# jinlong17/DA-Detect

Measured on AMD Instinct MI355X. Metric: train images/sec, DA-Faster-RCNN R-50 Cityscapes->Foggy, higher is better.
Workload: dtype f32

## Files before the change

### da_detect_amd/_C.py

```python
import contextlib
import os
import ctypes
import time

import torch

from . import _lib
from . import amax as _amax
from ._lib import ConvDesc

CL = torch.channels_last

NMS_TIE_RULE = 0

PROFILER = None
_KNAME_CACHE = {}


class KernelProfiler(object):

    def __init__(self, pool=0, only=None):
        self.only = only
        self._pool = []
        for _ in range(pool):
# ... 831 lines not shown
    R, C, h, w = x.shape
    y = torch.empty((R, C), dtype=torch.float32, device=x.device)
    _lib.call("dadet_avgpool_forward", _p(x), _p(y), R, h * w, C, _stream())
    return _amax.carry(y, x)


def avgpool_backward(gy, h, w):
    _dev(gy, "gy")
    gy = gy.contiguous()
    R, C = gy.shape
    gx = torch.empty((R, C, h, w), dtype=torch.float32, device=gy.device, memory_format=CL)
    _lib.call("dadet_avgpool_backward", _p(gy), _p(gx), R, h * w, C, _stream())
    return _amax.carry(gx, gy)


def nchw3_to_nhwc4(x):
    _dev(x, "x")
    x = x.contiguous()
    N, C, H, W = x.shape
    assert C == 3
    y = torch.empty((N, 4, H, W), dtype=torch.float32, device=x.device, memory_format=CL)
    _lib.call("dadet_nchw3_to_nhwc4", _p(x), _p(y), N, H, W, _stream())
    if _mode4():
        _amax.ptr(x)
        _amax.carry(y, x)
    return y


def two_image_ends(r_cst, n_src):
    return min(max(int(n_src), 0), int(r_cst)), int(r_cst)
# ... 303 lines not shown
        _lib.call("dadet_fpn_merge_levels", arr, len(chunk), _stream())
    return outs


def fast_rcnn_loss(class_logits, box_regression, src, labels_src, rows_pos, map_inds, targets_pos):
    _dev(class_logits, "class_logits"), _dev(box_regression, "box_regression")
    cls, reg = class_logits.contiguous(), box_regression.contiguous()
    losses = torch.empty(2, dtype=torch.float32, device=cls.device)
    g_cls, g_reg = torch.zeros_like(cls), torch.zeros_like(reg)
    _lib.call("dadet_fast_rcnn_loss", _p(cls), _p(reg), cls.shape[1], reg.shape[1], _p(src.contiguous()),
              _p(labels_src.contiguous()), int(src.numel()), _p(rows_pos.contiguous()), _p(map_inds.contiguous()),
              _p(targets_pos.contiguous()), int(rows_pos.numel()), _p(losses), _p(g_cls), _p(g_reg), _stream())
    return losses, g_cls, g_reg


def fast_rcnn_loss_rows(class_logits, box_regression, loss_labels, regression_targets):
    _dev(class_logits, "class_logits"), _dev(box_regression, "box_regression")
    cls, reg = class_logits.contiguous(), box_regression.contiguous()
    R = cls.shape[0]
    if loss_labels.numel() != R or regression_targets.numel() != 4 * R or reg.shape[0] != R:
        raise _lib.DadetError("fast_rcnn_loss_rows: %d logit rows, %d labels, %d target values" % (
            R, loss_labels.numel(), regression_targets.numel()))
    losses = torch.empty(2, dtype=torch.float32, device=cls.device)
    g_cls, g_reg = torch.zeros_like(cls), torch.zeros_like(reg)
    _lib.call("dadet_fast_rcnn_loss_rows", _p(cls), _p(reg), R, cls.shape[1], reg.shape[1],
              _p(loss_labels.contiguous().to(torch.int64)), _p(_dev(regression_targets, "targets").contiguous()),
              _p(losses), _p(g_cls), _p(g_reg), _stream())
    return losses, g_cls, g_reg


SAMPLE_ROIS_MAX = 4096
PROPOSALS_SAMPLE_MAX_GT = 1024


def sample_rois_buffers(rows, device):
    return dict(idx=torch.empty(rows, dtype=torch.int64, device=device),
                objectness=torch.empty(rows, dtype=torch.float32, device=device),
                boxes=torch.empty((rows, 4), dtype=torch.float32, device=device),
                labels=torch.empty(rows, dtype=torch.int64, device=device),
# ... 331 lines not shown
```

### da_detect_amd/_lib.py

```python
import ctypes
import os
from ctypes import POINTER, c_char_p, c_float, c_int, c_int64, c_size_t, c_uint64, c_void_p

_HERE = os.path.dirname(os.path.abspath(__file__))
LIB_PATH = os.environ.get("DADET_LIB") or os.path.join(_HERE, "libdadet_hip.so")
_lib = None
DEFAULT_GEMM_MODE = "4"


class ConvDesc(ctypes.Structure):

    _fields_ = [(n, c_int) for n in (
        "N", "H", "W", "Cin", "Cout", "KH", "KW", "stride", "pad", "Ho", "Wo", "OutH", "OutW",
        "out_spatial_stride", "relu_mode")]


class ConvPlanInfo(ctypes.Structure):

    _fields_ = [(n, c_int) for n in (
        "family", "variant", "tiles_m", "tiles_n", "ksplit", "splits", "rows_per_split", "sk_dp_tiles", "sk_tiles", "sk_units",
        "sk_iters", "sk_max_parts", "big_splits", "big_body", "launches", "grid", "needs_counters")] + [
        ("workspace_bytes", c_size_t), ("name", ctypes.c_char * 64)]


# ... 127 lines not shown
    "dadet_roi_pool_backward": [_P, _P, _P, _P, c_int, c_int, c_int, c_int, c_int, c_int, c_int, _P],
    "dadet_deform_psroi_pool_forward": [_P, _P, _P, _P, _P, c_int, c_int, c_int, c_int, c_int, c_int, c_float,
                                        c_int, c_int, c_int, c_int, c_int, c_float, c_int, _P],
    "dadet_deform_psroi_pool_backward": [_P, _P, _P, _P, _P, _P, _P, c_int, c_int, c_int, c_int, c_int, c_int,
                                         c_float, c_int, c_int, c_int, c_int, c_int, c_float, c_int, _P],
    "dadet_relu_bn_backward": [_P, _P, _P, _P, _P, c_int64, c_int, _P],
    "dadet_relu_bn_backward_m": [_P, _P, _P, _P, _P, c_int64, c_int, _P, _P, _P],
    "dadet_colsum_workspace_bytes": [c_int64, c_int, POINTER(c_size_t)],
    "dadet_colsum": [_P, _P, c_int64, c_int, _P, c_size_t, _P],
    "dadet_colsum_ld": [_P, c_int, _P, c_int64, c_int, c_int, _P, c_size_t, _P],
    "dadet_channel_affine": [_P, _P, _P, _P, c_int64, c_int, c_int, _P],
    "dadet_maxpool3x3s2_forward": [_P, _P, c_int, c_int, c_int, c_int, c_int, c_int, _P],
    "dadet_maxpool3x3s2_relu_backward": [_P, _P, _P, _P, c_int, c_int, c_int, c_int, c_int, c_int, _P, _P],
    "dadet_avgpool_forward": [_P, _P, c_int, c_int, c_int, _P],
    "dadet_avgpool_backward": [_P, _P, c_int, c_int, c_int, _P],
    "dadet_nchw3_to_nhwc4": [_P, _P, c_int, c_int, c_int, _P],
    "dadet_rpn_decode_clip": [_P, _P, _P, c_int, c_float, c_float, c_float, c_float, c_float, c_float, c_float, _P, _P],
    "dadet_da_img_head_loss_forward": [_P, _P, _P, _P, _P, _P, c_int, c_int, c_int, _P],
    "dadet_da_img_head_loss_backward": [_P, _P, _P, _P, _P, _P, _P, _P, _P, c_int, c_int, c_int, _P],
    "dadet_da_img_head_loss_backward_g": [_P, _P, _P, _P, _P, _P, _P, c_float, c_float, _P, _P, _P, _P, c_int, c_int, c_int,
                                          _P],
    "dadet_da_img_head_loss_backward_gm": [_P, _P, _P, _P, _P, _P, _P, c_float, c_float, _P, _P, _P, _P, c_int, c_int, c_int,
                                          _P, _P, _P],
    "dadet_da_ins_tail_forward": [_P, _P, _P, _P, _P, _P, _P, c_int, c_int, c_int, c_int, c_int, _P],
    "dadet_da_ins_tail_backward": [_P, _P, _P, _P, _P, _P, c_float, _P, _P, _P, _P, c_int, c_int, c_int, c_int, c_int, _P],
    "dadet_da_ins_tail_forward_n": [_P, _P, _P, _P, _P, _P, _P, c_int, c_int, POINTER(c_int), c_int, c_int, c_int, _P],
    "dadet_da_ins_tail_backward_n": [_P, _P, _P, _P, _P, _P, c_float, _P, _P, _P, _P, c_int, c_int, POINTER(c_int), c_int,
                                     c_int, c_int, _P],
    "dadet_da_ins_dropout_rows": [_P, _P, _P, c_int64, c_int, _P],
    "dadet_da_ins_merge": [_P, _P, _P, _P, _P, _P, c_int64, c_int, _P],
# ... 45 lines not shown
```

### da_detect_amd/csrc/elementwise.hip

```cpp
#include "box_match.h"
#include "conv_common.h"
#include <float.h>

namespace dadet {

static inline int stream_blocks(int64_t work_items, int threads) {
  int64_t b = ceil_div64(work_items, threads);
  if (b > kMaxStreamBlocks) b = kMaxStreamBlocks;
  if (b < 1) b = 1;
  return (int)b;
}

__global__ void relu_bn_backward_kernel(const float4* __restrict__ g, const float4* __restrict__ y,
                                        const float4* __restrict__ scale, float4* __restrict__ g_out,
                                        float4* __restrict__ g_scaled, int64_t total4, int C4,
                                        unsigned* __restrict__ amax_out, unsigned* __restrict__ amax_scaled) {
  float mo = 0.f, ms = 0.f;
  for (int64_t i = (int64_t)blockIdx.x * blockDim.x + threadIdx.x; i < total4;
       i += (int64_t)gridDim.x * blockDim.x) {
    const float4 gv = g[i];
    float4 r = gv;
    if (y) {
      const float4 yv = y[i];
      r.x = yv.x > 0.f ? gv.x : 0.f;
      r.y = yv.y > 0.f ? gv.y : 0.f;
      r.z = yv.z > 0.f ? gv.z : 0.f;
      r.w = yv.w > 0.f ? gv.w : 0.f;
    }
    if (g_out) g_out[i] = r;
    mo = fmaxf(fmaxf(mo, fmaxf(fabsf(r.x), fabsf(r.y))), fmaxf(fabsf(r.z), fabsf(r.w)));
    if (g_scaled) {
      float4 s = r;
      if (scale) {
        const float4 sc = scale[i % C4];
        s.x *= sc.x; s.y *= sc.y; s.z *= sc.z; s.w *= sc.w;
      }
      g_scaled[i] = s;
      ms = fmaxf(fmaxf(ms, fmaxf(fabsf(s.x), fabsf(s.y))), fmaxf(fabsf(s.z), fabsf(s.w)));
    }
  }
  if (amax_out) amax_publish(amax_out, mo);
  if (amax_scaled) amax_publish(amax_scaled, ms);
}

__global__ __launch_bounds__(256) void colsum_partial_kernel(const float* __restrict__ g,
                                                             float* __restrict__ partial, int64_t rows,
                                                             int C, int64_t rows_per_split, int cb, int ld) {
  __shared__ float red[256];
  const int lanes = 256 / cb;
// ... 422 lines not shown
  DADET_REQUIRE(rows >= 0 && C > 0 && C % 4 == 0, "relu_bn_backward: C=%d must be a multiple of 4", C);
  if (rows == 0) return DADET_OK;
  DADET_REQUIRE(g && (g_out || g_scaled), "relu_bn_backward: null pointer");
  DADET_REQUIRE(aligned16(g) && aligned16(y) && aligned16(scale) && aligned16(g_out) && aligned16(g_scaled),
                "relu_bn_backward: pointers must be 16-byte aligned");
  const int64_t total4 = rows * (C / 4);
  hipLaunchKernelGGL(relu_bn_backward_kernel, dim3(stream_blocks(total4, 256)), dim3(256), 0,
                     as_stream(stream), reinterpret_cast<const float4*>(g),
                     reinterpret_cast<const float4*>(y), reinterpret_cast<const float4*>(scale),
                     reinterpret_cast<float4*>(g_out), reinterpret_cast<float4*>(g_scaled), total4, C / 4,
                     reinterpret_cast<unsigned*>(g_out ? amax_out : nullptr),
                     reinterpret_cast<unsigned*>(g_scaled ? amax_scaled : nullptr));
  return check_launch("relu_bn_backward");
}

extern "C" int dadet_colsum_workspace_bytes(int64_t rows, int C, size_t* bytes_out) {
  DADET_REQUIRE(rows >= 0 && C > 0 && bytes_out, "colsum_workspace_bytes: bad args");
  *bytes_out = rows == 0 ? 0 : sizeof(float) * (size_t)colsum_splits(rows, C) * C;
  return DADET_OK;
}

extern "C" int dadet_colsum_ld(const float* g, int ld, float* out, int64_t rows, int C, int accumulate, void* workspace,
                               size_t workspace_bytes, void* stream) {
  DADET_REQUIRE(rows >= 0 && C > 0 && ld >= C && out, "colsum: bad args (rows=%lld C=%d ld=%d)", (long long)rows, C, ld);
  hipStream_t st = as_stream(stream);
  if (rows == 0) {
    if (!accumulate) (void)hipMemsetAsync(out, 0, sizeof(float) * C, st);
    return check_launch("colsum(empty)");
  }
  DADET_REQUIRE(g, "colsum: null input");
// ... 186 lines not shown
```

### da_detect_amd/layers/misc.py

```python

import torch
from torch import nn
from torch.autograd import Function
from torch.autograd.function import once_differentiable

from .. import _C
from .. import amax as _amax
from .conv import conv2d_affine_act

CL = torch.channels_last


class FrozenBatchNorm2d(nn.Module):

    def __init__(self, n):
        super(FrozenBatchNorm2d, self).__init__()
        self.register_buffer("weight", torch.ones(n))
        self.register_buffer("bias", torch.zeros(n))
        self.register_buffer("running_mean", torch.zeros(n))
        self.register_buffer("running_var", torch.ones(n))
        self._cache = None

    def folded(self):
        key = (self.weight._version, self.bias._version, self.running_mean._version,
# ... 278 lines not shown


class _AvgPoolHW(Function):

    @staticmethod
    def forward(ctx, x):
        ctx.hw = (x.shape[2], x.shape[3])
        return _C.avgpool_forward(x)

    @staticmethod
    @once_differentiable
    def backward(ctx, g):
        return _C.avgpool_backward(g, *ctx.hw)


_POOL_MEMO = True


def global_avg_pool(x):
    if x.shape[0] == 0:
        return x.new_empty((0, x.shape[1]))
    memo = x.__dict__.get("_dadet_pooled") if _POOL_MEMO else None
    if memo is not None and memo[0] == x._version and memo[1] == torch.is_grad_enabled():
        return memo[2]
    y = _AvgPoolHW.apply(x)
    x._dadet_pooled = (x._version, torch.is_grad_enabled(), y)
    return y
```

### da_detect_amd/modeling/backbone/resnet.py

```python
from collections import namedtuple

import torch
import torch.nn.functional as F
from torch import nn

from ... import _C
from ...layers import Conv2d, FrozenBatchNorm2d, conv2d_affine_act
from ...utils.registry import Registry
from ...utils import streams
from ...utils.streams import WgradLane

StageSpec = namedtuple("StageSpec", ["index", "block_count", "return_features"])


def _specs(*rows):
    return tuple(StageSpec(index=i, block_count=c, return_features=r) for (i, c, r) in rows)


ResNet50StagesTo5 = _specs((1, 3, False), (2, 4, False), (3, 6, False), (4, 3, True))
ResNet50StagesTo4 = _specs((1, 3, False), (2, 4, False), (3, 6, True))
ResNet101StagesTo5 = _specs((1, 3, False), (2, 4, False), (3, 23, False), (4, 3, True))
ResNet101StagesTo4 = _specs((1, 3, False), (2, 4, False), (3, 23, True))
ResNet50FPNStagesTo5 = _specs((1, 3, True), (2, 4, True), (3, 6, True), (4, 3, True))
ResNet101FPNStagesTo5 = _specs((1, 3, True), (2, 4, True), (3, 23, True), (4, 3, True))
# ... 30 lines not shown
        reqs, batch = self.reqs, self.batch
        key = self.key + tuple((tuple(r["x"].shape), r["stride"]) for r in reqs)

        def run():
            ok = self._known.get(key, True) and _C.conv_wgrad_group(reqs, batch)
            if not ok:
                self._known[key] = self._known[self.key] = False
                for r in reqs:
                    _C.conv_wgrad(r["x"], r["gy"], r["weight_shape"], r["stride"], r["pad"], out_scale=r["out_scale"],
                                  dw=r["dw"], accumulate=True, pending=batch)

        self.lane.run_group(run, *[t for r in reqs for t in (r["x"], r["gy"])])
        self.reqs = []


class _BlockBackward(object):

    def __init__(self, needs, x, w1, wd, s1, sd, stride):
        self.need_x, self.n1, self.n2, self.n3, nd = needs
        self.nd = nd and wd is not None
        self.x, self.w1, self.wd, self.s1, self.sd, self.stride = x, w1, wd, s1, sd, stride

    def open(self, G, out, out_private, y2, w2, w3, s3):
        self.S3 = G.contiguous(memory_format=torch.channels_last) if out_private else _C.relu_bn_backward(G, out, None)[1]
        self.lane = WgradLane(G.device, rows=G.shape[0] * G.shape[2] * G.shape[3])
        self.batch = _C.WgradBatch() if _WGRAD_BATCH else None
        weights = ((w3, self.n3), (w2, self.n2), (self.w1, self.n1), (self.wd, self.nd))
        self.group = _WgradGroup(self.lane, self.batch, [w for w, need in weights if need])
        dw3 = self.wgrad(w3, y2, self.S3, 1, 0, s3) if self.n3 else None
        return _C.conv_forward(self.S3, _C.conv_weight_transpose(w3, s3), relu_mode=2, mask_ref=y2), dw3

    def wgrad(self, w, xin, gout, st, pd, sc, shape=None, grouped=True):
        shape = tuple(w.shape) if shape is None else shape
        batch = self.batch
        if grouped and self.group.take(w, xin, gout, st, pd, sc, shape=shape):
            return None
        return self.lane.run_into(w, lambda acc: _C.conv_wgrad(xin, gout, shape, st, pd, out_scale=sc, dw=acc,
                                                               accumulate=True, pending=batch),
                                  lambda: _C.conv_wgrad(xin, gout, shape, st, pd, out_scale=sc, pending=batch),
# ... 440 lines not shown
```

### da_detect_amd/modeling/roi_heads/box_head/box_head.py

```python
import logging
import os

import torch

from ....structures.bounding_box import is_source_image
from ....utils import rng
from ...elision import elision_enabled, leading_source_images
from ....utils.streams import side_section
from .inference import make_roi_box_post_processor
from .loss import make_roi_box_loss_evaluator
from .roi_box_feature_extractors import make_roi_box_feature_extractor
from .roi_box_predictors import make_roi_box_predictor


_NO_DEDUP = os.environ.get("DADET_NO_ROI_DEDUP", "0") == "1"
_SPECULATE = os.environ.get("DADET_ROI_SPECULATE", "1") == "1"


class ROIBoxHead(torch.nn.Module):
    def __init__(self, cfg):
        super(ROIBoxHead, self).__init__()
        self.feature_extractor = make_roi_box_feature_extractor(cfg)
        self.predictor = make_roi_box_predictor(cfg)
        self.post_processor = make_roi_box_post_processor(cfg)
# ... 44 lines not shown
                    x = self.feature_extractor(features, state["speculative"])
                with torch.no_grad():
                    proposals = le.subsample_finish(state)
                    for _ in range(burn):
                        rng.next_seed(dev)
                    assert all(len(p) <= state["cap"] for p in proposals)
                    da_proposals = le.subsample_for_da(proposals, targets)
                if state["speculative"] is not None:
                    self._note_speculation(bool(state["exact"]))
                if not state["exact"]:
                    x = None
        else:
            x = None
        if x is None:
            x = self.feature_extractor(features, proposals)
        class_logits, box_regression = self.predictor(x)
        if not self.training:
            return x, self.post_processor((class_logits, box_regression), proposals), {}, x, None
        loss_classifier, loss_box_reg, _ = self.loss_evaluator([class_logits], [box_regression])
        if burn:
            return (x, proposals, dict(loss_classifier=loss_classifier, loss_box_reg=loss_box_reg), None, None)
        limit = self.loss_evaluator.fg_bg_sampler.batch_size_per_image
        same_set = all(len(p) <= limit for p in proposals) and not _NO_DEDUP
        if same_set:
            assert all(len(a) == len(b) for a, b in zip(da_proposals, proposals))
            da_ins_feas = x
        else:
            da_ins_feas = self.feature_extractor(features, da_proposals)
        da_ins_labels = torch.cat([p.get_field("domain_labels") for p in self.loss_evaluator._proposals], dim=0)
        da_ins_labels._n_src_host = sum(len(p) for p, t in zip(self.loss_evaluator._proposals, targets)
                                        if is_source_image(t))
        da_ins_labels._rows_per_image_host = tuple(len(p) for p in self.loss_evaluator._proposals)
        return (x, proposals, dict(loss_classifier=loss_classifier, loss_box_reg=loss_box_reg), da_ins_feas,
                da_ins_labels)
# ... 5 lines not shown
```

### da_detect_amd/modeling/roi_heads/box_head/loss.py

```python
import os

import torch
from torch.nn import functional as F

from .... import _C
from ....layers import smooth_l1_loss
from ....layers.misc import fast_rcnn_loss_fused, fast_rcnn_loss_rows_fused
from ....structures.bounding_box import BoxList, is_source_image
from ....structures.boxlist_ops import boxlist_iou
from ...balanced_positive_negative_sampler import BalancedPositiveNegativeSampler
from ...box_coder import BoxCoder
from ...matcher import Matcher
from ...utils import cat
from ....utils import rng



def _nz(mask, size):
    if _STATIC:
        return torch.nonzero_static(mask, size=size)
    return torch.nonzero(mask)


_STATIC = True
# ... 219 lines not shown
                    prop.add_field("domain_labels", torch.full((n,), bool(is_source), dtype=torch.bool, device=dev))
                out.append(prop)
                continue
            if counts is None:
                counts = torch.empty((len(proposals), 2), dtype=torch.int32, device=dev)
            s = _C.sample_rois(prop.bbox, None, None, cap, int(cap * sampler.positive_fraction), rng.next_seed(dev),
                               is_source, counts[len(out)])
            b = BoxList(s["boxes"], prop.size, prop.mode)
            for name in prop.fields():
                if name != "domain_labels":
                    b.add_field(name, prop.get_field(name)[s["idx"]])
            b.add_field("domain_labels", s["domain"])
            out.append(b)
        return out

    def __call__(self, class_logits, box_regression):
        class_logits = cat(class_logits, dim=0)
        box_regression = cat(box_regression, dim=0)
        if not hasattr(self, "_proposals"):
            raise RuntimeError("subsample needs to be called before")
        prep = self._loss_prep
        if prep.get("rows"):
            cls_loss, box_loss = fast_rcnn_loss_rows_fused(class_logits, box_regression, prep["loss_labels"],
                                                           prep["regression_targets"])
            return cls_loss, box_loss, prep["domain_masks"]
        labels = prep["labels_src"]
        if class_logits.is_cuda and not self.cls_agnostic_bbox_reg:
            cls_loss, box_loss = fast_rcnn_loss_fused(class_logits, box_regression, prep["src"], labels,
                                                      prep["rows_pos"].reshape(-1), prep["map_inds"],
                                                      prep["regression_targets_pos"])
            return cls_loss, box_loss, prep["domain_masks"]
        classification_loss = F.cross_entropy(class_logits.index_select(0, prep["src"]), labels)
        box_loss = smooth_l1_loss(box_regression[prep["rows_pos"], prep["map_inds"]], prep["regression_targets_pos"],
                                  size_average=False, beta=1)
        box_loss = box_loss / labels.numel()
        return classification_loss, box_loss, prep["domain_masks"]

# ... 9 lines not shown
```

### da_detect_amd/modeling/roi_heads/box_head/roi_box_predictors.py

```python
from torch import nn

from ....layers import conv1x1_multi, global_avg_pool
from ... import registry


class _TwoLinearPredictor(nn.Module):
    def _build(self, cfg, in_features):
        classes = cfg.MODEL.ROI_BOX_HEAD.NUM_CLASSES
        box_classes = 2 if cfg.MODEL.CLS_AGNOSTIC_BBOX_REG else classes
        self.cls_score = nn.Linear(in_features, classes)
        self.bbox_pred = nn.Linear(in_features, 4 * box_classes)
        for layer, std in ((self.cls_score, 0.01), (self.bbox_pred, 0.001)):
            nn.init.normal_(layer.weight, mean=0, std=std)
            nn.init.constant_(layer.bias, 0)

    def _predict(self, vectors):
        rows = vectors.shape[0]
        scores, deltas = conv1x1_multi(vectors.reshape(rows, -1, 1, 1),
                                       [self.cls_score.weight, self.bbox_pred.weight],
                                       [self.cls_score.bias, self.bbox_pred.bias])
        return scores.reshape(rows, -1), deltas.reshape(rows, -1)


@registry.ROI_BOX_PREDICTOR.register("FastRCNNPredictor")
class FastRCNNPredictor(_TwoLinearPredictor):

    def __init__(self, config, pretrained=None):
        super(FastRCNNPredictor, self).__init__()
        self.avgpool = nn.AvgPool2d(kernel_size=7, stride=7)
        self._build(config, config.MODEL.RESNETS.RES2_OUT_CHANNELS * 8)

    def forward(self, x):
        if tuple(x.shape[2:]) != (7, 7):
            raise ValueError("FastRCNNPredictor expects 7x7 ROI features, got %s" % (tuple(x.shape),))
        return self._predict(global_avg_pool(x))


@registry.ROI_BOX_PREDICTOR.register("FPNPredictor")
class FPNPredictor(_TwoLinearPredictor):

    def __init__(self, cfg):
        super(FPNPredictor, self).__init__()
        self._build(cfg, cfg.MODEL.ROI_BOX_HEAD.MLP_HEAD_DIM)

    def forward(self, x):
        return self._predict(x)


def make_roi_box_predictor(cfg):
    return registry.ROI_BOX_PREDICTOR[cfg.MODEL.ROI_BOX_HEAD.PREDICTOR](cfg)
```

### include/dadet.h

```cpp
#ifndef DADET_H_
#define DADET_H_

#include <stddef.h>
#include <stdint.h>

#ifdef __cplusplus
extern "C" {
#endif

#define DADET_OK 0
#define DADET_EINVAL (-1)
#define DADET_ELAUNCH (-2)
#define DADET_EWORKSPACE (-3)
#define DADET_EUNSUPPORTED (-4)

const char* dadet_last_error(void);
int dadet_version(void);
int dadet_device_info(int* cu_count, int* clock_khz, size_t* hbm_bytes, char* arch_name, int arch_name_len);

int dadet_nms_workspace_bytes(int n, size_t* bytes_out);
int dadet_nms(const float* boxes_xyxy, const float* scores, int n, float thresh, int tie_rule,
              int max_keep, void* workspace, size_t workspace_bytes, int64_t* keep_out,
              int* num_keep_out, void* stream);
int dadet_nms_batch_workspace_bytes(int batch, int n_max, size_t* bytes_out);
// ... 281 lines not shown
int dadet_relu_bn_backward_m(const float* g, const float* y, const float* scale, float* g_out, float* g_scaled,
                             int64_t rows, int C, float* amax_out, float* amax_scaled, void* stream);
int dadet_colsum_workspace_bytes(int64_t rows, int C, size_t* bytes_out);
int dadet_colsum_ld(const float* g, int ld, float* out, int64_t rows, int C, int accumulate, void* workspace,
                    size_t workspace_bytes, void* stream);
int dadet_colsum(const float* g, float* out, int64_t rows, int C, void* workspace, size_t workspace_bytes,
                 void* stream);
int dadet_channel_affine(const float* x, const float* scale, const float* bias, float* y, int64_t rows,
                         int C, int relu, void* stream);
int dadet_maxpool3x3s2_forward(const float* x, float* y, int N, int H, int W, int C, int Ho, int Wo,
                               void* stream);
int dadet_maxpool3x3s2_relu_backward(const float* y, const float* gp, const float* scale, float* g, int N, int H,
                                     int W, int C, int Ho, int Wo, float* amax_out, void* stream);
int dadet_avgpool_forward(const float* x, float* y, int R, int HW, int C, void* stream);
int dadet_avgpool_backward(const float* gy, float* gx, int R, int HW, int C, void* stream);
int dadet_nchw3_to_nhwc4(const float* x, float* y, int N, int H, int W, void* stream);

int dadet_rpn_decode_clip(const float* deltas, const float* anchors, const int64_t* topk_idx, int K,
                          float wx, float wy, float ww, float wh, float xform_clip, float im_w,
                          float im_h, float* boxes_out, void* stream);

int dadet_da_img_head_loss_forward(const float* t, const float* w2, const float* b2, const float* labels,
                                   float* logits_out, float* sums_out, int num_images,
                                   int rows_per_image, int C1, void* stream);
int dadet_da_img_head_loss_backward(const float* t, const float* w2, const float* logits,
                                    const float* labels, const float* coef, float* g_t_w, float* g_t_x,
                                    float* g_w2, float* g_b2, int num_images, int rows_per_image, int C1,
                                    void* stream);
int dadet_da_img_head_loss_backward_g(const float* t, const float* w2, const float* logits, const float* labels,
                                      const float* g_bce, const float* g_mean_sig, const float* w_adv_dev, float w_adv,
// ... 44 lines not shown
```

Before: 163.0.

## Fuse ROI box-head avgpool, predictor linears and loss gradients into custom kernels

```diff
diff --git a/da_detect_amd/_C.py b/da_detect_amd/_C.py
--- a/da_detect_amd/_C.py
+++ b/da_detect_amd/_C.py
@@ -869,6 +869,85 @@
     return _amax.carry(gx, gy)
 
 
+def unpool_relu_bn_backward(gy, y, scale=None, want_unscaled=False, div=None):
+    _dev(gy, "gy"), _dev(y, "y")
+    gy, y = gy.contiguous(), _nhwc(y)
+    R, C, h, w = y.shape
+    assert tuple(gy.shape) == (R, C), "unpool_relu_bn_backward: gy %s for y %s" % (tuple(gy.shape), tuple(y.shape))
+    g_out = torch.empty_like(y) if want_unscaled else None
+    g_scaled = torch.empty_like(y)
+    so = ss = None
+    if _mode4():
+        if g_out is not None and _amax.slot_of(_amax.carry(g_out, gy)) is None:
+            so = _amax.new_slot(y.device)
+        if scale is not None or _amax.slot_of(_amax.carry(g_scaled, gy)) is None:
+            ss = _amax.new_slot(y.device)
+    _lib.call("dadet_unpool_relu_bn_backward_m", _p(gy), _p(y), _p(scale), _p(g_out), _p(g_scaled), R, h * w, C,
+              float(h * w if div is None else div), ctypes.c_void_p(so[0]) if so else None,
+              ctypes.c_void_p(ss[0]) if ss else None, _stream())
+    if so:
+        _amax.attach(g_out, so)
+    if ss:
+        _amax.attach(g_scaled, ss)
+    return g_out, g_scaled
+
+
+BOX_TAIL = os.environ.get("DADET_BOX_TAIL", "1") == "1"
+BOX_TAIL_MAX_C, BOX_TAIL_MAX_COLS, BOX_TAIL_MAX_HW = 4096, 128, 64
+
+
+def box_tail_supported(hw, C, n_cls, n_reg):
+    return (1 <= hw <= BOX_TAIL_MAX_HW and C % 256 == 0 and 0 < C <= BOX_TAIL_MAX_C and n_cls >= 1 and n_reg >= 1
+            and n_cls + n_reg <= BOX_TAIL_MAX_COLS)
+
+
+def _rowmajor(t, name):
+    return _dev(t, name).detach().contiguous()
+
+
+def box_tail_forward(x, w_cls, b_cls, w_reg, b_reg, loss_grads=False):
+    x = _nhwc(_dev(x, "x"))
+    R, C, h, w = x.shape
+    w_cls, w_reg = _rowmajor(w_cls, "w_cls"), _rowmajor(w_reg, "w_reg")
+    n_cls, n_reg = w_cls.shape[0], w_reg.shape[0]
+    assert w_cls.shape[1] == C and w_reg.shape[1] == C and b_cls.numel() == n_cls and b_reg.numel() == n_reg
+    pooled = torch.empty((R, C), dtype=torch.float32, device=x.device)
+    cls = torch.empty((R, n_cls), dtype=torch.float32, device=x.device)
+    reg = torch.empty((R, n_reg), dtype=torch.float32, device=x.device)
+    zc, zr = (torch.empty_like(cls), torch.empty_like(reg)) if loss_grads else (None, None)
+    _lib.call("dadet_box_tail_forward", _p(x), _p(w_cls), _p(_rowmajor(b_cls, "b_cls")), _p(w_reg),
+              _p(_rowmajor(b_reg, "b_reg")), _p(pooled), _p(cls), _p(reg), _p(zc), _p(zr), R, h * w, C, n_cls, n_reg,
+              _stream())
+    if loss_grads:
+        return _amax.carry(pooled, x), cls, reg, (zc, zr)
+    return _amax.carry(pooled, x), cls, reg
+
+
+def box_tail_backward(g_cls, g_reg, g0, g1, pooled, w_cls, w_reg, hw, g2=None, into=None):
+    g_cls, g_reg, pooled = _dev(g_cls, "g_cls").contiguous(), _dev(g_reg, "g_reg").contiguous(), pooled.contiguous()
+    w_cls, w_reg = _rowmajor(w_cls, "w_cls"), _rowmajor(w_reg, "w_reg")
+    R, C = pooled.shape
+    n_cls, n_reg = w_cls.shape[0], w_reg.shape[0]
+    assert tuple(g_cls.shape) == (R, n_cls) and tuple(g_reg.shape) == (R, n_reg)
+    g0, g1 = _dev(g0, "g0").contiguous(), _dev(g1, "g1").contiguous()
+    assert g0.numel() == 1 and g1.numel() == 1
+    if g2 is not None:
+        g2 = _dev(g2, "g2").contiguous()
+        assert tuple(g2.shape) == (R, C)
+    d_pooled = torch.empty((R, C), dtype=torch.float32, device=pooled.device)
+    if into is None:
+        outs = (torch.empty_like(w_cls), torch.empty(n_cls, dtype=torch.float32, device=pooled.device),
+                torch.empty_like(w_reg), torch.empty(n_reg, dtype=torch.float32, device=pooled.device))
+    else:
+        outs = tuple(into)
+        assert all(o.is_contiguous() and o.dtype == torch.float32 for o in outs)
+        assert [o.numel() for o in outs] == [n_cls * C, n_cls, n_reg * C, n_reg]
+    _lib.call("dadet_box_tail_backward", _p(g_cls), _p(g_reg), _p(g0), _p(g1), _p(pooled), _p(w_cls), _p(w_reg), _p(g2),
+              _p(d_pooled), _p(outs[0]), _p(outs[1]), _p(outs[2]), _p(outs[3]), R, int(hw), C, n_cls, n_reg,
+              0 if into is None else 1, _stream())
+    return d_pooled, outs
+
+
 def nchw3_to_nhwc4(x):
     _dev(x, "x")
     x = x.contiguous()
@@ -1202,7 +1281,7 @@
     return losses, g_cls, g_reg
 
 
-def fast_rcnn_loss_rows(class_logits, box_regression, loss_labels, regression_targets):
+def fast_rcnn_loss_rows(class_logits, box_regression, loss_labels, regression_targets, grads=None):
     _dev(class_logits, "class_logits"), _dev(box_regression, "box_regression")
     cls, reg = class_logits.contiguous(), box_regression.contiguous()
     R = cls.shape[0]
@@ -1210,7 +1289,8 @@
         raise _lib.DadetError("fast_rcnn_loss_rows: %d logit rows, %d labels, %d target values" % (
             R, loss_labels.numel(), regression_targets.numel()))
     losses = torch.empty(2, dtype=torch.float32, device=cls.device)
-    g_cls, g_reg = torch.zeros_like(cls), torch.zeros_like(reg)
+    g_cls, g_reg = (torch.zeros_like(cls), torch.zeros_like(reg)) if grads is None else grads
+    assert g_cls.shape == cls.shape and g_reg.shape == reg.shape and g_cls.is_contiguous() and g_reg.is_contiguous()
     _lib.call("dadet_fast_rcnn_loss_rows", _p(cls), _p(reg), R, cls.shape[1], reg.shape[1],
               _p(loss_labels.contiguous().to(torch.int64)), _p(_dev(regression_targets, "targets").contiguous()),
               _p(losses), _p(g_cls), _p(g_reg), _stream())
diff --git a/da_detect_amd/_lib.py b/da_detect_amd/_lib.py
--- a/da_detect_amd/_lib.py
+++ b/da_detect_amd/_lib.py
@@ -165,6 +165,10 @@
     "dadet_maxpool3x3s2_relu_backward": [_P, _P, _P, _P, c_int, c_int, c_int, c_int, c_int, c_int, _P, _P],
     "dadet_avgpool_forward": [_P, _P, c_int, c_int, c_int, _P],
     "dadet_avgpool_backward": [_P, _P, c_int, c_int, c_int, _P],
+    "dadet_unpool_relu_bn_backward_m": [_P, _P, _P, _P, _P, c_int, c_int, c_int, c_float, _P, _P, _P],
+    "dadet_box_tail_forward": [_P, _P, _P, _P, _P, _P, _P, _P, _P, _P, c_int, c_int, c_int, c_int, c_int, _P],
+    "dadet_box_tail_backward": [_P, _P, _P, _P, _P, _P, _P, _P, _P, _P, _P, _P, _P, c_int, c_int, c_int, c_int, c_int, c_int,
+                                _P],
     "dadet_nchw3_to_nhwc4": [_P, _P, c_int, c_int, c_int, _P],
     "dadet_rpn_decode_clip": [_P, _P, _P, c_int, c_float, c_float, c_float, c_float, c_float, c_float, c_float, _P, _P],
     "dadet_da_img_head_loss_forward": [_P, _P, _P, _P, _P, _P, c_int, c_int, c_int, _P],
diff --git a/da_detect_amd/csrc/box_tail.hip b/da_detect_amd/csrc/box_tail.hip
--- /dev/null
+++ b/da_detect_amd/csrc/box_tail.hip
@@ -0,0 +1,264 @@
+#include "common.h"
+
+namespace dadet {
+
+constexpr int kBoxTailMaxC = 4096;
+constexpr int kBoxTailMaxCols = 128;
+constexpr int kBoxTailMaxHW = 64;
+
+__device__ inline float4 f4_zero() { return make_float4(0.f, 0.f, 0.f, 0.f); }
+__device__ inline void f4_add(float4& a, const float4 v) { a.x += v.x; a.y += v.y; a.z += v.z; a.w += v.w; }
+__device__ inline void f4_mad(float4& a, const float4 w, const float4 p) {
+  a.x += w.x * p.x; a.y += w.y * p.y; a.z += w.z * p.z; a.w += w.w * p.w;
+}
+__device__ inline void f4_smad(float4& a, const float s, const float4 w) {
+  a.x += s * w.x; a.y += s * w.y; a.z += s * w.z; a.w += s * w.w;
+}
+
+__global__ __launch_bounds__(512) void box_tail_forward_kernel(const float4* __restrict__ x, const float4* __restrict__ wc,
+                                                               const float* __restrict__ bc, const float4* __restrict__ wr,
+                                                               const float* __restrict__ br, int HW, int C4, int n_cls,
+                                                               int n_reg, float4* __restrict__ pooled,
+                                                               float* __restrict__ cls, float* __restrict__ reg,
+                                                               float* __restrict__ zero_cls, float* __restrict__ zero_reg) {
+  __shared__ float4 s_pool[kBoxTailMaxC / 4];
+  const int r = blockIdx.x;
+  if (zero_cls)
+    for (int n = threadIdx.x; n < n_cls; n += 512) zero_cls[(size_t)r * n_cls + n] = 0.f;
+  if (zero_reg)
+    for (int n = threadIdx.x; n < n_reg; n += 512) zero_reg[(size_t)r * n_reg + n] = 0.f;
+  const float4* xr = x + (size_t)r * HW * C4;
+  const float inv = (float)HW;
+  for (int c = threadIdx.x; c < C4; c += 512) {
+    float4 a = f4_zero();
+    int p = 0;
+    for (; p + 8 <= HW; p += 8) {
+      float4 v[8];
+#pragma unroll
+      for (int u = 0; u < 8; ++u) v[u] = xr[(size_t)(p + u) * C4 + c];
+#pragma unroll
+      for (int u = 0; u < 8; ++u) f4_add(a, v[u]);
+    }
+    for (; p < HW; ++p) f4_add(a, xr[(size_t)p * C4 + c]);
+    a.x /= inv; a.y /= inv; a.z /= inv; a.w /= inv;
+    s_pool[c] = a;
+    pooled[(size_t)r * C4 + c] = a;
+  }
+  __syncthreads();
+  const int wave = threadIdx.x >> 6, lane = threadIdx.x & 63;
+  const int N = n_cls + n_reg;
+  for (int n0 = wave; n0 < N; n0 += 32) {
+    const float4* w[4];
+#pragma unroll
+    for (int j = 0; j < 4; ++j) {
+      const int n = min(n0 + 8 * j, N - 1);
+      w[j] = n < n_cls ? wc + (size_t)n * C4 : wr + (size_t)(n - n_cls) * C4;
+    }
+    float4 acc[4] = {f4_zero(), f4_zero(), f4_zero(), f4_zero()};
+#pragma unroll 2
+    for (int c = lane; c < C4; c += 64) {
+      const float4 pv = s_pool[c];
+#pragma unroll
+      for (int j = 0; j < 4; ++j) f4_mad(acc[j], w[j][c], pv);
+    }
+#pragma unroll
+    for (int j = 0; j < 4; ++j) {
+      float s = (acc[j].x + acc[j].y) + (acc[j].z + acc[j].w);
+#pragma unroll
+      for (int o = 32; o > 0; o >>= 1) s += __shfl_xor(s, o, 64);
+      const int n = n0 + 8 * j;
+      if (lane == 0 && n < N) {
+        if (n < n_cls) cls[(size_t)r * n_cls + n] = s + bc[n];
+        else reg[(size_t)r * n_reg + (n - n_cls)] = s + br[n - n_cls];
+      }
+    }
+  }
+}
+
+__global__ __launch_bounds__(256) void box_tail_backward_kernel(
+    const float* __restrict__ g_cls, const float* __restrict__ g_reg, const float* __restrict__ g0p,
+    const float* __restrict__ g1p, const float* __restrict__ pooled, const float* __restrict__ wc,
+    const float* __restrict__ wr, const float* __restrict__ g2, float* __restrict__ d_pooled, float* __restrict__ dwc,
+    float* __restrict__ dbc, float* __restrict__ dwr, float* __restrict__ dbr, int R, float div, int C, int n_cls,
+    int n_reg, int accumulate) {
+  __shared__ __attribute__((aligned(16))) float s_g[256 * 8];
+  __shared__ float s_red[4 * 8 * 64];
+  __shared__ float s_redb[4 * 8];
+  __shared__ int s_cnt;
+  const int N = n_cls + n_reg;
+  const float g0 = g0p[0], g1 = g1p[0];
+  const int wave = threadIdx.x >> 6, lane = threadIdx.x & 63;
+  if ((int)blockIdx.x < R) {
+    const int r = blockIdx.x;
+    float* s_val = s_g;
+    int* s_idx = reinterpret_cast<int*>(s_g + 136);
+    if (wave == 0) {
+      int cnt = 0;
+      for (int h = 0; h < 2; ++h) {
+        const int n = h * 64 + lane;
+        float v = 0.f;
+        if (n < n_cls) v = g_cls[(size_t)r * n_cls + n] * g0;
+        else if (n < N) v = g_reg[(size_t)r * n_reg + (n - n_cls)] * g1;
+        const unsigned long long m = __ballot(v != 0.f);
+        if (v != 0.f) {
+          const int at = cnt + __popcll(m & ((1ull << lane) - 1ull));
+          s_val[at] = v;
+          s_idx[at] = n;
+        }
+        cnt += __popcll(m);
+      }
+      const int padded = (cnt + 7) & ~7;
+      if (lane < padded - cnt) {
+        s_val[cnt + lane] = 0.f;
+        s_idx[cnt + lane] = 0;
+      }
+      if (lane == 0) s_cnt = padded;
+    }
+    __syncthreads();
+    const int cnt = s_cnt;
+    const int C4 = C >> 2;
+    const float4* wc4 = reinterpret_cast<const float4*>(wc);
+    const float4* wr4 = reinterpret_cast<const float4*>(wr);
+    for (int c = threadIdx.x; c < C4; c += 256) {
+      float4 acc[4] = {f4_zero(), f4_zero(), f4_zero(), f4_zero()};
+      for (int i = 0; i < cnt; i += 8) {
+        float4 w[8];
+#pragma unroll
+        for (int u = 0; u < 8; ++u) {
+          const int n = s_idx[i + u];
+          w[u] = n < n_cls ? wc4[(size_t)n * C4 + c] : wr4[(size_t)(n - n_cls) * C4 + c];
+        }
+#pragma unroll
+        for (int u = 0; u < 8; ++u) f4_smad(acc[u & 3], s_val[i + u], w[u]);
+      }
+      float4 d;
+      d.x = (acc[0].x + acc[1].x) + (acc[2].x + acc[3].x);
+      d.y = (acc[0].y + acc[1].y) + (acc[2].y + acc[3].y);
+      d.z = (acc[0].z + acc[1].z) + (acc[2].z + acc[3].z);
+      d.w = (acc[0].w + acc[1].w) + (acc[2].w + acc[3].w);
+      if (g2) f4_add(d, reinterpret_cast<const float4*>(g2)[(size_t)r * C4 + c]);
+      d.x /= div; d.y /= div; d.z /= div; d.w /= div;
+      reinterpret_cast<float4*>(d_pooled)[(size_t)r * C4 + c] = d;
+    }
+    return;
+  }
+  const int b = blockIdx.x - R;
+  const int slabs = C >> 6;
+  const int slab = b % slabs, n0 = (b / slabs) * 8;
+  const int ch = slab * 64 + lane;
+  float acc[8][8], accb[8][8];
+#pragma unroll
+  for (int u = 0; u < 8; ++u)
+#pragma unroll
+    for (int j = 0; j < 8; ++j) acc[u][j] = accb[u][j] = 0.f;
+  for (int r0 = 0; r0 < R; r0 += 256) {
+    {
+      const int r = r0 + threadIdx.x;
+#pragma unroll
+      for (int j = 0; j < 8; ++j) {
+        const int n = n0 + j;
+        float v = 0.f;
+        if (r < R) {
+          if (n < n_cls) v = g_cls[(size_t)r * n_cls + n] * g0;
+          else if (n < N) v = g_reg[(size_t)r * n_reg + (n - n_cls)] * g1;
+        }
+        s_g[threadIdx.x * 8 + j] = v;
+      }
+    }
+    __syncthreads();
+    const int first = r0 + wave * 64;
+    const int rows = min(64, R - first);
+    const float* prow = pooled + (size_t)first * C + ch;
+    for (int i0 = 0; i0 < rows; i0 += 8) {
+      float p[8];
+#pragma unroll
+      for (int u = 0; u < 8; ++u) p[u] = i0 + u < rows ? prow[(size_t)(i0 + u) * C] : 0.f;
+#pragma unroll
+      for (int u = 0; u < 8; ++u) {
+        if (i0 + u >= rows) break;
+        const float4 ga = *reinterpret_cast<const float4*>(&s_g[(wave * 64 + i0 + u) * 8]);
+        const float4 gb = *reinterpret_cast<const float4*>(&s_g[(wave * 64 + i0 + u) * 8 + 4]);
+        acc[u][0] += ga.x * p[u]; acc[u][1] += ga.y * p[u]; acc[u][2] += ga.z * p[u]; acc[u][3] += ga.w * p[u];
+        acc[u][4] += gb.x * p[u]; acc[u][5] += gb.y * p[u]; acc[u][6] += gb.z * p[u]; acc[u][7] += gb.w * p[u];
+        if (slab == 0) {
+          accb[u][0] += ga.x; accb[u][1] += ga.y; accb[u][2] += ga.z; accb[u][3] += ga.w;
+          accb[u][4] += gb.x; accb[u][5] += gb.y; accb[u][6] += gb.z; accb[u][7] += gb.w;
+        }
+      }
+    }
+    __syncthreads();
+  }
+#pragma unroll
+  for (int j = 0; j < 8; ++j) {
+    s_red[(wave * 8 + j) * 64 + lane] =
+        ((acc[0][j] + acc[1][j]) + (acc[2][j] + acc[3][j])) + ((acc[4][j] + acc[5][j]) + (acc[6][j] + acc[7][j]));
+    if (lane == 0)
+      s_redb[wave * 8 + j] =
+          ((accb[0][j] + accb[1][j]) + (accb[2][j] + accb[3][j])) + ((accb[4][j] + accb[5][j]) + (accb[6][j] + accb[7][j]));
+  }
+  __syncthreads();
+  for (int j = wave; j < 8; j += 4) {
+    const int n = n0 + j;
+    if (n >= N) continue;
+    const float s = (s_red[(0 * 8 + j) * 64 + lane] + s_red[(1 * 8 + j) * 64 + lane]) +
+                    (s_red[(2 * 8 + j) * 64 + lane] + s_red[(3 * 8 + j) * 64 + lane]);
+    float* dst = n < n_cls ? dwc + (size_t)n * C + ch : dwr + (size_t)(n - n_cls) * C + ch;
+    *dst = accumulate ? *dst + s : s;
+  }
+  if (slab == 0 && threadIdx.x < 8 && n0 + (int)threadIdx.x < N) {
+    const int j = threadIdx.x, n = n0 + j;
+    const float s = (s_redb[0 * 8 + j] + s_redb[1 * 8 + j]) + (s_redb[2 * 8 + j] + s_redb[3 * 8 + j]);
+    float* dst = n < n_cls ? dbc + n : dbr + (n - n_cls);
+    *dst = accumulate ? *dst + s : s;
+  }
+}
+
+}
+
+using namespace dadet;
+
+static bool aligned16(const void* p) { return (reinterpret_cast<uintptr_t>(p) & 15) == 0; }
+
+static int box_tail_check_shape(const char* who, int R, int HW, int C, int n_cls, int n_reg) {
+  DADET_REQUIRE(R >= 0 && HW >= 1 && HW <= kBoxTailMaxHW, "%s: R=%d HW=%d outside 0 <= R, 1 <= HW <= %d", who, R, HW,
+                kBoxTailMaxHW);
+  DADET_REQUIRE(C > 0 && C % 256 == 0 && C <= kBoxTailMaxC, "%s: C=%d must be a multiple of 256 up to %d", who, C,
+                kBoxTailMaxC);
+  DADET_REQUIRE(n_cls >= 1 && n_reg >= 1 && n_cls + n_reg <= kBoxTailMaxCols,
+                "%s: %d classes + %d regression columns outside 1 .. %d", who, n_cls, n_reg, kBoxTailMaxCols);
+  return DADET_OK;
+}
+
+extern "C" int dadet_box_tail_forward(const float* x, const float* w_cls, const float* b_cls, const float* w_reg,
+                                      const float* b_reg, float* pooled, float* class_logits, float* box_regression,
+                                      float* zero_cls, float* zero_reg, int R, int HW, int C, int n_cls, int n_reg,
+                                      void* stream) {
+  const int rc = box_tail_check_shape("box_tail_forward", R, HW, C, n_cls, n_reg);
+  if (rc != DADET_OK) return rc;
+  if (R == 0) return DADET_OK;
+  DADET_REQUIRE(x && w_cls && b_cls && w_reg && b_reg && pooled && class_logits && box_regression,
+                "box_tail_forward: null pointer");
+  DADET_REQUIRE(aligned16(x) && aligned16(w_cls) && aligned16(w_reg) && aligned16(pooled),
+                "box_tail_forward: x, the weights and pooled must be 16-byte aligned");
+  hipLaunchKernelGGL(box_tail_forward_kernel, dim3(R), dim3(512), 0, as_stream(stream),
+                     reinterpret_cast<const float4*>(x), reinterpret_cast<const float4*>(w_cls), b_cls,
+                     reinterpret_cast<const float4*>(w_reg), b_reg, HW, C / 4, n_cls, n_reg,
+                     reinterpret_cast<float4*>(pooled), class_logits, box_regression, zero_cls, zero_reg);
+  return check_launch("box_tail_forward");
+}
+
+extern "C" int dadet_box_tail_backward(const float* g_cls, const float* g_reg, const float* g0, const float* g1,
+                                       const float* pooled, const float* w_cls, const float* w_reg, const float* g2,
+                                       float* d_pooled, float* dw_cls, float* db_cls, float* dw_reg, float* db_reg, int R,
+                                       int HW, int C, int n_cls, int n_reg, int accumulate, void* stream) {
+  const int rc = box_tail_check_shape("box_tail_backward", R, HW, C, n_cls, n_reg);
+  if (rc != DADET_OK) return rc;
+  DADET_REQUIRE(g0 && g1 && w_cls && w_reg && dw_cls && db_cls && dw_reg && db_reg, "box_tail_backward: null pointer");
+  DADET_REQUIRE(R == 0 || (g_cls && g_reg && pooled && d_pooled), "box_tail_backward: null pointer");
+  DADET_REQUIRE(aligned16(w_cls) && aligned16(w_reg) && aligned16(g2) && aligned16(d_pooled),
+                "box_tail_backward: the weights, g2 and d_pooled must be 16-byte aligned");
+  const int blocks = R + (C / 64) * ceil_div(n_cls + n_reg, 8);
+  hipLaunchKernelGGL(box_tail_backward_kernel, dim3(blocks), dim3(256), 0, as_stream(stream), g_cls, g_reg, g0, g1, pooled,
+                     w_cls, w_reg, g2, d_pooled, dw_cls, db_cls, dw_reg, db_reg, R, (float)HW, C, n_cls, n_reg, accumulate);
+  return check_launch("box_tail_backward");
+}
diff --git a/da_detect_amd/csrc/elementwise.hip b/da_detect_amd/csrc/elementwise.hip
--- a/da_detect_amd/csrc/elementwise.hip
+++ b/da_detect_amd/csrc/elementwise.hip
@@ -33,6 +33,41 @@
       float4 s = r;
       if (scale) {
         const float4 sc = scale[i % C4];
+        s.x *= sc.x; s.y *= sc.y; s.z *= sc.z; s.w *= sc.w;
+      }
+      g_scaled[i] = s;
+      ms = fmaxf(fmaxf(ms, fmaxf(fabsf(s.x), fabsf(s.y))), fmaxf(fabsf(s.z), fabsf(s.w)));
+    }
+  }
+  if (amax_out) amax_publish(amax_out, mo);
+  if (amax_scaled) amax_publish(amax_scaled, ms);
+}
+
+__global__ void unpool_relu_bn_backward_kernel(const float4* __restrict__ gy, const float4* __restrict__ y,
+                                               const float4* __restrict__ scale, float4* __restrict__ g_out,
+                                               float4* __restrict__ g_scaled, int64_t total4, int HW, int C4, float div,
+                                               unsigned* __restrict__ amax_out, unsigned* __restrict__ amax_scaled) {
+  float mo = 0.f, ms = 0.f;
+  for (int64_t i = (int64_t)blockIdx.x * blockDim.x + threadIdx.x; i < total4;
+       i += (int64_t)gridDim.x * blockDim.x) {
+    const int c = (int)(i % C4);
+    const int64_t row = i / ((int64_t)HW * C4);
+    float4 gv = gy[row * C4 + c];
+    gv.x /= div; gv.y /= div; gv.z /= div; gv.w /= div;
+    float4 r = gv;
+    if (y) {
+      const float4 yv = y[i];
+      r.x = yv.x > 0.f ? gv.x : 0.f;
+      r.y = yv.y > 0.f ? gv.y : 0.f;
+      r.z = yv.z > 0.f ? gv.z : 0.f;
+      r.w = yv.w > 0.f ? gv.w : 0.f;
+    }
+    if (g_out) g_out[i] = r;
+    mo = fmaxf(fmaxf(mo, fmaxf(fabsf(r.x), fabsf(r.y))), fmaxf(fabsf(r.z), fabsf(r.w)));
+    if (g_scaled) {
+      float4 s = r;
+      if (scale) {
+        const float4 sc = scale[c];
         s.x *= sc.x; s.y *= sc.y; s.z *= sc.z; s.w *= sc.w;
       }
       g_scaled[i] = s;
@@ -485,6 +520,25 @@
   return check_launch("relu_bn_backward");
 }
 
+extern "C" int dadet_unpool_relu_bn_backward_m(const float* gy, const float* y, const float* scale, float* g_out,
+                                               float* g_scaled, int R, int HW, int C, float div, float* amax_out,
+                                               float* amax_scaled, void* stream) {
+  DADET_REQUIRE(R >= 0 && HW > 0 && C > 0 && C % 4 == 0, "unpool_relu_bn_backward: bad dims (R=%d HW=%d C=%d)", R, HW, C);
+  DADET_REQUIRE(div > 0.f, "unpool_relu_bn_backward: div must be positive");
+  if (R == 0) return DADET_OK;
+  DADET_REQUIRE(gy && (g_out || g_scaled), "unpool_relu_bn_backward: null pointer");
+  DADET_REQUIRE(aligned16(gy) && aligned16(y) && aligned16(scale) && aligned16(g_out) && aligned16(g_scaled),
+                "unpool_relu_bn_backward: pointers must be 16-byte aligned");
+  const int64_t total4 = (int64_t)R * HW * (C / 4);
+  hipLaunchKernelGGL(unpool_relu_bn_backward_kernel, dim3(stream_blocks(total4, 256)), dim3(256), 0, as_stream(stream),
+                     reinterpret_cast<const float4*>(gy), reinterpret_cast<const float4*>(y),
+                     reinterpret_cast<const float4*>(scale), reinterpret_cast<float4*>(g_out),
+                     reinterpret_cast<float4*>(g_scaled), total4, HW, C / 4, div,
+                     reinterpret_cast<unsigned*>(g_out ? amax_out : nullptr),
+                     reinterpret_cast<unsigned*>(g_scaled ? amax_scaled : nullptr));
+  return check_launch("unpool_relu_bn_backward");
+}
+
 extern "C" int dadet_colsum_workspace_bytes(int64_t rows, int C, size_t* bytes_out) {
   DADET_REQUIRE(rows >= 0 && C > 0 && bytes_out, "colsum_workspace_bytes: bad args");
   *bytes_out = rows == 0 ? 0 : sizeof(float) * (size_t)colsum_splits(rows, C) * C;
diff --git a/da_detect_amd/layers/misc.py b/da_detect_amd/layers/misc.py
--- a/da_detect_amd/layers/misc.py
+++ b/da_detect_amd/layers/misc.py
@@ -316,6 +316,80 @@
         return _C.avgpool_backward(g, *ctx.hw)
 
 
+def _grad_slot(param):
+    from ..utils import streams
+
+    if not streams.DIRECT_WGRAD or not isinstance(param, torch.Tensor) or not param.is_leaf or not param.requires_grad:
+        return None
+    g = param.grad
+    if g is None or not g.is_cuda or g.dtype != torch.float32 or g.shape != param.shape or not g.is_contiguous():
+        return None
+    return g
+
+
+class _BoxTail(Function):
+
+    @staticmethod
+    def forward(ctx, x, w_cls, b_cls, w_reg, b_reg, loss_labels, regression_targets, started):
+        pooled, cls, reg, grads = started.outputs
+        losses, g_cls, g_reg = _C.fast_rcnn_loss_rows(cls, reg, loss_labels, regression_targets, grads=grads)
+        ctx.save_for_backward(pooled, g_cls, g_reg, w_cls, w_reg)
+        ctx.params = (w_cls, b_cls, w_reg, b_reg)
+        ctx.x_shape = tuple(x.shape)
+        ctx.set_materialize_grads(False)
+        return pooled, losses[0], losses[1]
+
+    @staticmethod
+    @once_differentiable
+    def backward(ctx, g_pooled, g0, g1):
+        pooled, g_cls, g_reg, w_cls, w_reg = ctx.saved_tensors
+        R, C, h, w = ctx.x_shape
+        zero = None
+        if g0 is None or g1 is None:
+            zero = torch.zeros((), dtype=torch.float32, device=pooled.device)
+        slots = [_grad_slot(p) for p in ctx.params]
+        direct = all(s is not None for s in slots) and all(ctx.needs_input_grad[1:5])
+        d_pooled, grads = _C.box_tail_backward(g_cls, g_reg, zero if g0 is None else g0, zero if g1 is None else g1,
+                                               pooled, w_cls, w_reg, h * w, g2=g_pooled, into=slots if direct else None)
+        dx = d_pooled.view(R, C, 1, 1).expand(R, C, h, w) if ctx.needs_input_grad[0] else None
+        if direct:
+            return (dx,) + (None,) * 7
+        return (dx,) + tuple(g if need else None for g, need in zip(grads, ctx.needs_input_grad[1:5])) + (None, None, None)
+
+
+def box_tail_supported(x, w_cls, w_reg):
+    return (_C.BOX_TAIL and torch.is_grad_enabled() and x.is_cuda and x.dtype == torch.float32 and x.dim() == 4
+            and x.shape[0] > 0 and w_cls.dim() == 2 and w_cls.shape[1] == x.shape[1]
+            and _C.box_tail_supported(x.shape[2] * x.shape[3], x.shape[1], w_cls.shape[0], w_reg.shape[0]))
+
+
+class BoxTailStarted(object):
+
+    def __init__(self, x, params, outputs):
+        self.x, self.params, self.outputs = x, params, outputs
+        self.cls, self.reg = outputs[1], outputs[2]
+        self.finished = False
+
+
+def box_tail_start(x, w_cls, b_cls, w_reg, b_reg):
+    with torch.no_grad():
+        outputs = _C.box_tail_forward(x, w_cls, b_cls, w_reg, b_reg, loss_grads=True)
+    started = BoxTailStarted(x, (w_cls, b_cls, w_reg, b_reg), outputs)
+    started.cls._dadet_box_tail = started
+    return started
+
+
+def box_tail_finish(started, loss_labels, regression_targets):
+    x = started.x
+    pooled, cls_loss, box_loss = _BoxTail.apply(x, *started.params, loss_labels, regression_targets, started)
+    if _POOL_MEMO:
+        x._dadet_pooled = (x._version, torch.is_grad_enabled(), pooled)
+    started.finished = True
+    started.outputs = started.x = None
+    started.cls.__dict__.pop("_dadet_box_tail", None)
+    return cls_loss, box_loss
+
+
 _POOL_MEMO = True
 
 
diff --git a/da_detect_amd/modeling/backbone/resnet.py b/da_detect_amd/modeling/backbone/resnet.py
--- a/da_detect_amd/modeling/backbone/resnet.py
+++ b/da_detect_amd/modeling/backbone/resnet.py
@@ -68,6 +68,15 @@
         self.reqs = []
 
 
+def _unpooled_rows(G):
+    if not _C.BOX_TAIL or G.dim() != 4 or not G.is_cuda or G.dtype != torch.float32:
+        return None
+    R, C, h, w = G.shape
+    if R == 0 or h * w == 1 or C % 4 or G.stride() != (C, 1, 0, 0) or G.data_ptr() % 16:
+        return None
+    return G[:, :, 0, 0]
+
+
 class _BlockBackward(object):
 
     def __init__(self, needs, x, w1, wd, s1, sd, stride):
@@ -76,7 +85,11 @@
         self.x, self.w1, self.wd, self.s1, self.sd, self.stride = x, w1, wd, s1, sd, stride
 
     def open(self, G, out, out_private, y2, w2, w3, s3):
-        self.S3 = G.contiguous(memory_format=torch.channels_last) if out_private else _C.relu_bn_backward(G, out, None)[1]
+        rows = None if out_private else _unpooled_rows(G)
+        if rows is not None:
+            self.S3 = _C.unpool_relu_bn_backward(rows, out, None, div=1.0)[1]
+        else:
+            self.S3 = G.contiguous(memory_format=torch.channels_last) if out_private else _C.relu_bn_backward(G, out, None)[1]
         self.lane = WgradLane(G.device, rows=G.shape[0] * G.shape[2] * G.shape[3])
         self.batch = _C.WgradBatch() if _WGRAD_BATCH else None
         weights = ((w3, self.n3), (w2, self.n2), (self.w1, self.n1), (self.wd, self.nd))
diff --git a/da_detect_amd/modeling/roi_heads/box_head/box_head.py b/da_detect_amd/modeling/roi_heads/box_head/box_head.py
--- a/da_detect_amd/modeling/roi_heads/box_head/box_head.py
+++ b/da_detect_amd/modeling/roi_heads/box_head/box_head.py
@@ -82,10 +82,15 @@
             x = None
         if x is None:
             x = self.feature_extractor(features, proposals)
-        class_logits, box_regression = self.predictor(x)
+        started = None
+        if self.training and hasattr(self.predictor, "tail_start"):
+            started = self.predictor.tail_start(x, self.loss_evaluator.row_targets())
+        class_logits, box_regression = (started.cls, started.reg) if started is not None else self.predictor(x)
         if not self.training:
             return x, self.post_processor((class_logits, box_regression), proposals), {}, x, None
         loss_classifier, loss_box_reg, _ = self.loss_evaluator([class_logits], [box_regression])
+        if started is not None and not started.finished:
+            raise RuntimeError("box head: the loss evaluator did not complete the fused tail (its logits carry no graph)")
         if burn:
             return (x, proposals, dict(loss_classifier=loss_classifier, loss_box_reg=loss_box_reg), None, None)
         limit = self.loss_evaluator.fg_bg_sampler.batch_size_per_image
diff --git a/da_detect_amd/modeling/roi_heads/box_head/loss.py b/da_detect_amd/modeling/roi_heads/box_head/loss.py
--- a/da_detect_amd/modeling/roi_heads/box_head/loss.py
+++ b/da_detect_amd/modeling/roi_heads/box_head/loss.py
@@ -5,7 +5,7 @@
 
 from .... import _C
 from ....layers import smooth_l1_loss
-from ....layers.misc import fast_rcnn_loss_fused, fast_rcnn_loss_rows_fused
+from ....layers.misc import box_tail_finish, fast_rcnn_loss_fused, fast_rcnn_loss_rows_fused
 from ....structures.bounding_box import BoxList, is_source_image
 from ....structures.boxlist_ops import boxlist_iou
 from ...balanced_positive_negative_sampler import BalancedPositiveNegativeSampler
@@ -257,6 +257,12 @@
             out.append(b)
         return out
 
+    def row_targets(self):
+        prep = getattr(self, "_loss_prep", None)
+        if not prep or not prep.get("rows"):
+            return None
+        return prep["loss_labels"], prep["regression_targets"]
+
     def __call__(self, class_logits, box_regression):
         class_logits = cat(class_logits, dim=0)
         box_regression = cat(box_regression, dim=0)
@@ -264,6 +270,10 @@
             raise RuntimeError("subsample needs to be called before")
         prep = self._loss_prep
         if prep.get("rows"):
+            started = class_logits.__dict__.get("_dadet_box_tail")
+            if started is not None and started.reg is box_regression and not started.finished:
+                cls_loss, box_loss = box_tail_finish(started, prep["loss_labels"], prep["regression_targets"])
+                return cls_loss, box_loss, prep["domain_masks"]
             cls_loss, box_loss = fast_rcnn_loss_rows_fused(class_logits, box_regression, prep["loss_labels"],
                                                            prep["regression_targets"])
             return cls_loss, box_loss, prep["domain_masks"]
diff --git a/da_detect_amd/modeling/roi_heads/box_head/roi_box_predictors.py b/da_detect_amd/modeling/roi_heads/box_head/roi_box_predictors.py
--- a/da_detect_amd/modeling/roi_heads/box_head/roi_box_predictors.py
+++ b/da_detect_amd/modeling/roi_heads/box_head/roi_box_predictors.py
@@ -1,6 +1,7 @@
 from torch import nn
 
 from ....layers import conv1x1_multi, global_avg_pool
+from ....layers.misc import box_tail_start, box_tail_supported
 from ... import registry
 
 
@@ -35,6 +36,12 @@
             raise ValueError("FastRCNNPredictor expects 7x7 ROI features, got %s" % (tuple(x.shape),))
         return self._predict(global_avg_pool(x))
 
+    def tail_start(self, x, row_targets):
+        if row_targets is None or tuple(x.shape[2:]) != (7, 7) or x.shape[0] != row_targets[0].numel() \
+                or not box_tail_supported(x, self.cls_score.weight, self.bbox_pred.weight):
+            return None
+        return box_tail_start(x, self.cls_score.weight, self.cls_score.bias, self.bbox_pred.weight, self.bbox_pred.bias)
+
 
 @registry.ROI_BOX_PREDICTOR.register("FPNPredictor")
 class FPNPredictor(_TwoLinearPredictor):
diff --git a/include/dadet.h b/include/dadet.h
--- a/include/dadet.h
+++ b/include/dadet.h
@@ -319,6 +319,16 @@
                                      int W, int C, int Ho, int Wo, float* amax_out, void* stream);
 int dadet_avgpool_forward(const float* x, float* y, int R, int HW, int C, void* stream);
 int dadet_avgpool_backward(const float* gy, float* gx, int R, int HW, int C, void* stream);
+int dadet_unpool_relu_bn_backward_m(const float* gy, const float* y, const float* scale, float* g_out, float* g_scaled,
+                                    int R, int HW, int C, float div, float* amax_out, float* amax_scaled, void* stream);
+
+int dadet_box_tail_forward(const float* x, const float* w_cls, const float* b_cls, const float* w_reg, const float* b_reg,
+                           float* pooled, float* class_logits, float* box_regression, float* zero_cls, float* zero_reg,
+                           int R, int HW, int C, int n_cls, int n_reg, void* stream);
+int dadet_box_tail_backward(const float* g_cls, const float* g_reg, const float* g0, const float* g1, const float* pooled,
+                            const float* w_cls, const float* w_reg, const float* g2, float* d_pooled, float* dw_cls,
+                            float* db_cls, float* dw_reg, float* db_reg, int R, int HW, int C, int n_cls, int n_reg,
+                            int accumulate, void* stream);
 int dadet_nchw3_to_nhwc4(const float* x, float* y, int N, int H, int W, void* stream);
 
 int dadet_rpn_decode_clip(const float* deltas, const float* anchors, const int64_t* topk_idx, int K,
```

Result: faster. 164.7 (median of 6 runs) (+1.0%).
